# gildas-lormeau/zlib-streams-ts

Measured on AMD Instinct MI355X. Metric: uncompressed MB/s, deflate-raw L6, 4096x64KiB batch at 1/2/4/8 GPUs, higher is better.
Workload: dtype u8; 1 GPU; 4096 x 65536 B text-corpus streams split across the GPUs, deflate-raw level 6; global_streams=4096, streams_per_gpu=4096, stream_bytes=65536, level=6, format=deflate-raw, compressed_bytes=91855591, parallelism=dp1

## Files before the change

### zlib-streams-ts_amd/csrc/deflate_sweep.hip

```cpp
#include <hip/hip_runtime.h>
#include "zs_common.h"
#include "zs_kernels.h"
#include <type_traits>

#define ZS_SW_WIN_WORDS ((ZS_SEG_WPOS + 258u + 20u + 3u) / 4u + 2u)
#define ZS_SW_RING 128u
#ifndef ZS_SW_EXP
#define ZS_SW_EXP 0
#endif
#define ZS_SW_MW 320u

typedef __attribute__((address_space(3))) uint32_t zs_sw_lds_u32;
static __device__ __forceinline__ uint32_t sw_lds_addr(const void* p) {
  return (uint32_t)(uintptr_t)(const zs_sw_lds_u32*)p;
}

static __device__ __forceinline__ uint32_t sw_hash(uint32_t w) {
  return (((w & 0xffu) << 10) ^ (((w >> 8) & 0xffu) << 5) ^ ((w >> 16) & 0xffu)) & ZS_HASH_MASK;
}

#define ZS_BK_WPT (16384u / ZS_BK_THREADS)
#define ZS_BK_PPL (ZS_BK_THREADS / 64u)
#ifndef ZS_BK_PROF
#define ZS_BK_PROF 0
#endif
#if ZS_BK_PROF
__device__ unsigned long long zs_bk_stat[4];
extern "C" int zs_bucket_stats(unsigned long long* out) {
  return (int)hipMemcpyFromSymbol(out, HIP_SYMBOL(zs_bk_stat), sizeof(zs_bk_stat));
}
#define BK_MARK(i) do { if (threadIdx.x == 0) { const unsigned long long t_ = wall_clock64(); atomicAdd(&zs_bk_stat[i], t_ - bk_t); bk_t = t_; } } while (0)
#else
#define BK_MARK(i) do { } while (0)
#endif
#define ZS_BK_INFLIGHT 8
#define ZS_BK_CHUNK 2048u

template <bool ORD>
__global__ __launch_bounds__(ZS_BK_THREADS) void zs_k_bucket(const uint8_t* __restrict__ in,
                                                            const uint64_t* __restrict__ in_off,
                                                            const uint32_t* __restrict__ in_len,
                                                            const uint64_t* __restrict__ pos_base,
                                                            const zs_sweep_seg* __restrict__ segs,
                                                            uint16_t* __restrict__ members, uint2* __restrict__ mres) {
  __shared__ uint32_t cnt[16384];
  __shared__ uint32_t part[ZS_BK_THREADS];
  __shared__ uint32_t stg[ZS_BK_CHUNK / 4 + 2];
  __shared__ uint16_t q[2][ZS_BK_CHUNK];
  const zs_sweep_seg G = segs[blockIdx.x];
  const int s = (int)G.s;
  const uint32_t nrel = in_len[s] - G.base;
  const uint32_t tid = threadIdx.x;
  const uint8_t* src = in + in_off[s] + G.base;
  uint16_t* mem = members + G.mb;
  uint2* out = mres + pos_base[s] + G.base;
  const uint32_t m = nrel > 2 ? min(nrel - 2, G.ohi) : 0u;
  const uint32_t n = min(nrel, m + 2u);
  if (nrel - m <= 2u)
    for (uint32_t p = m + tid; p < nrel; p += ZS_BK_THREADS) out[p] = make_uint2(0, 0);
  if (m == 0) return;
  for (uint32_t i = tid; i < 16384 / 4; i += ZS_BK_THREADS) reinterpret_cast<uint4*>(cnt)[i] = make_uint4(0, 0, 0, 0);
  const bool aligned = ((uintptr_t)src & 3u) == 0;
#if ZS_BK_PROF
  unsigned long long bk_t = wall_clock64();
  if (threadIdx.x == 0) atomicAdd(&zs_bk_stat[3], 1ull);
#endif
  __syncthreads();
  {
    uint32_t w[5], nw[5];
    auto load5 = [&](uint32_t p0, uint32_t* x) __attribute__((always_inline)) {
#pragma unroll
      for (int k = 0; k < 5; k++) x[k] = zs_load_word(src, n, p0 + 16 * tid + 4 * k);
    };
    load5(0, nw);
    for (uint32_t p0 = 0; p0 < m; p0 += 16 * ZS_BK_THREADS) {
#pragma unroll
      for (int k = 0; k < 5; k++) w[k] = nw[k];
      if (p0 + 16 * ZS_BK_THREADS < m) load5(p0 + 16 * ZS_BK_THREADS, nw);
#pragma unroll
      for (uint32_t j = 0; j < 16; j++) {
        const uint32_t p = p0 + 16 * tid + j;
        const uint32_t h = sw_hash(__builtin_amdgcn_alignbyte(w[(j >> 2) + 1], w[j >> 2], j & 3u));
        if (p < m) atomicAdd(&cnt[h >> 1], 1u << (16u * (h & 1u)));
      }
    }
  }
  __syncthreads();
  BK_MARK(0);
  {
    uint32_t sum = 0;
    for (uint32_t j = 0; j < ZS_BK_WPT; j++) {
      const uint32_t w = cnt[ZS_BK_WPT * tid + ((j + tid) & (ZS_BK_WPT - 1u))];
      sum += (w & 0xffffu) + (w >> 16);
    }
    part[tid] = sum;
    __syncthreads();
    if (tid < 64) {
      uint32_t v[ZS_BK_PPL], t = 0;
#pragma unroll
      for (uint32_t j = 0; j < ZS_BK_PPL; j++) { v[j] = part[ZS_BK_PPL * tid + j]; t += v[j]; }
      uint32_t x = t;
#pragma unroll
      for (int d = 1; d < 64; d <<= 1) {
        const uint32_t y = __shfl_up(x, d, 64);
        if (tid >= (uint32_t)d) x += y;
      }
      uint32_t run = x - t;
#pragma unroll
      for (uint32_t j = 0; j < ZS_BK_PPL; j++) { part[ZS_BK_PPL * tid + j] = run; run += v[j]; }
    }
    __syncthreads();
    uint32_t run = part[tid];
    for (uint32_t j = 0; j < ZS_BK_WPT; j++) {
      const uint32_t w = cnt[ZS_BK_WPT * tid + j];
      const uint32_t lo = w & 0xffffu;
      cnt[ZS_BK_WPT * tid + j] = run | ((run + lo) << 16);
      run += lo + (w >> 16);
    }
  }
  __syncthreads();
  BK_MARK(1);
  const uint32_t wave = tid >> 6, lane = tid & 63u;
  constexpr uint32_t CW = ZS_BK_CHUNK / 4 / 64;
  uint32_t nxt[CW + 1];
  auto fetch = [&](uint32_t c0) {
#pragma unroll
    for (uint32_t i = 0; i <= CW; i++) {
      const uint32_t w = 64 * i + lane;
      const uint32_t at = c0 + 4 * w;
      uint32_t v = 0;
      if (w < ZS_BK_CHUNK / 4 + 2) {
        if (aligned && at + 4 <= n) v = *(const uint32_t*)(src + at);
        else
          for (uint32_t k = 0; k < 4; k++)
            if (at + k < n) v |= (uint32_t)src[at + k] << (8 * k);
      }
      nxt[i] = v;
    }
  };
  if (wave == 0) fetch(0);
  const uint32_t nch = (m + ZS_BK_CHUNK - 1) / ZS_BK_CHUNK;
  for (uint32_t c = 0; c <= nch; c++) {
    const uint32_t c0 = c * ZS_BK_CHUNK;
    if (wave == 0 && c < nch) {
      __builtin_amdgcn_s_waitcnt(0xc07f);
      __builtin_amdgcn_wave_barrier();
#pragma unroll
      for (uint32_t i = 0; i <= CW; i++)
        if (64 * i + lane < ZS_BK_CHUNK / 4 + 2) stg[64 * i + lane] = nxt[i];
      __builtin_amdgcn_s_waitcnt(0xc07f);
      __builtin_amdgcn_wave_barrier();
      if (c0 + ZS_BK_CHUNK < m) fetch(c0 + ZS_BK_CHUNK);
      const uint32_t c1 = min(m, c0 + ZS_BK_CHUNK);
      uint16_t* const qc = q[c & 1u];
      for (uint32_t g0 = c0; g0 < c1; g0 += 64 * ZS_BK_INFLIGHT) {
        uint32_t a[ZS_BK_INFLIGHT], v[ZS_BK_INFLIGHT], sh[ZS_BK_INFLIGHT], e[ZS_BK_INFLIGHT], hh[ZS_BK_INFLIGHT];
#pragma unroll
        for (int j = 0; j < ZS_BK_INFLIGHT; j++) {
          const uint32_t p = g0 + 64 * j + lane;
          const uint32_t o = p - c0;
          const uint32_t h = sw_hash(__builtin_amdgcn_alignbyte(stg[(o >> 2) + 1], stg[o >> 2], o & 3u));
          hh[j] = h;
          sh[j] = 16u * (h & 1u);
          a[j] = sw_lds_addr(&cnt[h >> 1]);
          v[j] = p < c1 ? 1u << sh[j] : 0u;
        }
        if (!ORD) {
#pragma unroll
          for (int j = 0; j < ZS_BK_INFLIGHT; j++) {
            const uint32_t p = g0 + 64 * j + lane;
            const uint32_t h = hh[j];
            const uint64_t mm = zs_wave_match(h, p < c1);
            const uint32_t rank = (uint32_t)__builtin_popcountll(mm & ((1ull << lane) - 1ull));
            const uint32_t lead = mm ? (uint32_t)__builtin_ctzll(mm) : lane;
            uint32_t old = 0;
            if (p < c1 && lead == lane)
              old = atomicAdd(&cnt[h >> 1], (uint32_t)__builtin_popcountll(mm) << sh[j]);
            old = (uint32_t)__builtin_amdgcn_ds_bpermute((int)(lead * 4u), (int)old);
            e[j] = old + (rank << sh[j]);
          }
        } else {
        asm volatile(
            "ds_add_rtn_u32 %0, %8, %16\n\t"
            "ds_add_rtn_u32 %1, %9, %17\n\t"
            "ds_add_rtn_u32 %2, %10, %18\n\t"
            "ds_add_rtn_u32 %3, %11, %19\n\t"
            "ds_add_rtn_u32 %4, %12, %20\n\t"
            "ds_add_rtn_u32 %5, %13, %21\n\t"
            "ds_add_rtn_u32 %6, %14, %22\n\t"
            "ds_add_rtn_u32 %7, %15, %23\n\t"
            "s_waitcnt lgkmcnt(0)"
            : "=&v"(e[0]), "=&v"(e[1]), "=&v"(e[2]), "=&v"(e[3]), "=&v"(e[4]), "=&v"(e[5]), "=&v"(e[6]), "=&v"(e[7])
            : "v"(a[0]), "v"(a[1]), "v"(a[2]), "v"(a[3]), "v"(a[4]), "v"(a[5]), "v"(a[6]), "v"(a[7]), "v"(v[0]),
              "v"(v[1]), "v"(v[2]), "v"(v[3]), "v"(v[4]), "v"(v[5]), "v"(v[6]), "v"(v[7])
            : "memory");
        }
#pragma unroll
        for (int j = 0; j < ZS_BK_INFLIGHT; j++) {
          const uint32_t p = g0 + 64 * j + lane;
          if (p < c1) qc[p - c0] = (uint16_t)(e[j] >> sh[j]);
        }
      }
    } else if (wave != 0 && c > 0) {
      const uint32_t b0 = c0 - ZS_BK_CHUNK, cnt1 = min(m, c0) - b0;
      const uint16_t* const qp = q[(c - 1) & 1u];
      for (uint32_t o = tid - 64u; o < cnt1; o += ZS_BK_THREADS - 64u) mem[qp[o]] = (uint16_t)(b0 + o);
    }
    __syncthreads();
  }
  BK_MARK(2);
}
template __global__ void zs_k_bucket<true>(const uint8_t*, const uint64_t*, const uint32_t*, const uint64_t*,
                                           const zs_sweep_seg*, uint16_t*, uint2*);
template __global__ void zs_k_bucket<false>(const uint8_t*, const uint64_t*, const uint32_t*, const uint64_t*,
                                            const zs_sweep_seg*, uint16_t*, uint2*);

static __device__ __forceinline__ uint32_t sw_word(const uint32_t* win, uint32_t off) {
  const uint32_t i = off >> 2;
  return __builtin_amdgcn_alignbyte(win[i + 1], win[i], off & 3u);
}

static __device__ __forceinline__ uint32_t sw_extend(const uint32_t* win, uint32_t p, uint32_t q, uint32_t maxc,
                                                     uint32_t from) {
  uint32_t k = from;
  while (k < maxc) {
    const uint32_t y = sw_word(win, q + k) ^ sw_word(win, p + k);
    if (y) { k += (uint32_t)(__builtin_ctz(y) >> 3); break; }
    k += 4;
  }
  return k < maxc ? k : maxc;
}

static __device__ __forceinline__ uint64_t sw_uniform(uint64_t x) {
  return ((uint64_t)(uint32_t)__builtin_amdgcn_readfirstlane((uint32_t)(x >> 32)) << 32) |
         (uint64_t)(uint32_t)__builtin_amdgcn_readfirstlane((uint32_t)x);
}

static __device__ __forceinline__ uint32_t max3(uint32_t a, uint32_t b, uint32_t c) {
  return max(max(a, b), c);
}

static __device__ __forceinline__ uint32_t sw_x7(uint32_t w) {
  const uint32_t b0 = w & 0xffu, b1 = (w >> 8) & 0xffu;
  return ((b0 >> 5) & 3u) | ((b1 & 7u) << 2) | (((b1 >> 5) & 3u) << 5);
}
template <bool A7>
struct SwSig;
template <>
struct SwSig<false> {
  static constexpr uint32_t LONG = 88u;
  static constexpr uint32_t THR0 = 23u;
  static constexpr uint32_t EXT = 11u;
  uint32_t a, b, c;
  __device__ __forceinline__ void own(const uint32_t* win, uint32_t p) {
    a = sw_word(win, p);
    b = sw_word(win, p + 4);
    c = (sw_word(win, p + 8) & 0x00ffffffu) | 0x01000000u;
  }
  static __device__ __forceinline__ uint4 rec(const uint32_t* win, uint32_t q, uint32_t w0) {
    return make_uint4(w0, sw_word(win, q + 4), sw_word(win, q + 8) & 0x00ffffffu, 0u);
  }
  __device__ __forceinline__ uint32_t mbits(uint32_t x, uint32_t y, uint32_t z) const {
    uint32_t f0, f1, f2;
    asm("v_ffbl_b32 %0, %1" : "=v"(f0) : "v"(x ^ a));
    asm("v_ffbl_b32 %0, %1\n\tv_add_u32_e64 %0, %0, 32 clamp" : "=&v"(f1) : "v"(y ^ b));
    asm("v_ffbl_b32 %0, %1\n\tv_add_u32_e32 %0, 64, %0" : "=&v"(f2) : "v"(z ^ c));
    return min(min(f0, f1), f2);
  }
  static __device__ __forceinline__ uint32_t len(uint32_t sigma) { return sigma; }
};
template <>
struct SwSig<true> {
  static constexpr uint32_t LONG = 64u;
  static constexpr uint32_t THR0 = 7u;
  static constexpr uint32_t EXT = 10u;
  uint32_t a, b;
  __device__ __forceinline__ void own(const uint32_t* win, uint32_t p) {
    a = sw_x7(sw_word(win, p)) | (sw_word(win, p + 3) << 8);
    b = sw_word(win, p + 6);
  }
  static __device__ __forceinline__ uint4 rec(const uint32_t* win, uint32_t q, uint32_t w0) {
    return make_uint4(sw_x7(w0) | (sw_word(win, q + 3) << 8), sw_word(win, q + 6), sw_word(win, q + EXT), 0u);
  }
  __device__ __forceinline__ uint32_t mbits(uint32_t x, uint32_t y, uint32_t) const {
    uint32_t f0, f1;
    asm("v_ffbl_b32 %0, %1" : "=v"(f0) : "v"(x ^ a));
    asm("v_ffbl_b32 %0, %1\n\tv_add_u32_e64 %0, %0, 32 clamp" : "=&v"(f1) : "v"(y ^ b));
    return min(min(f0, f1), 64u);
  }
  static __device__ __forceinline__ uint32_t len(uint32_t sigma) { return sigma ? sigma + 2u : 2u; }
};

struct SwRing {
  uint2 ab[2 * ZS_SW_RING];
  uint32_t c[2 * ZS_SW_RING];
  uint32_t key[2 * ZS_SW_RING];
};

#if ZS_SW_EXP & 64
__device__ unsigned long long zs_sw_stat[8];
#define SW_STAT(i, v) do { if ((threadIdx.x & 63u) == __builtin_ctzll(__builtin_amdgcn_read_exec())) atomicAdd(&zs_sw_stat[i], (unsigned long long)(v)); } while (0)
extern "C" int zs_sw_stats(unsigned long long* out) {
  return (int)hipMemcpyFromSymbol(out, HIP_SYMBOL(zs_sw_stat), sizeof(zs_sw_stat));
}
#else
#define SW_STAT(i, v) do { } while (0)
#endif

template <bool A7, bool MW>
static __device__ __forceinline__ void sw_body(const uint32_t* win, SwRing* R, uint16_t* mw, uint32_t* next,
                                               uint32_t n, uint32_t m, uint32_t olo, uint32_t ohi,
                                               const uint16_t* mem, uint2* out, int chain, int nice_cfg) {
  using Sig = SwSig<A7>;
  const uint32_t lane = threadIdx.x & 63u;
  const uint32_t budget = (uint32_t)chain, budget_s = (uint32_t)chain >> 2;
#if ZS_SW_EXP & 128
  const uint32_t sbud = 4u;
#else
  const uint32_t sbud = budget;
#endif
  const uint32_t nchunks = (m + 63) / 64;
  auto put_rec = [&](int j, uint4 r) {
    const uint32_t i = (uint32_t)j & (ZS_SW_RING - 1);
    R->ab[i] = make_uint2(r.x, r.y);
    R->ab[i + ZS_SW_RING] = make_uint2(r.x, r.y);
    R->c[i] = r.z;
    R->c[i + ZS_SW_RING] = r.z;
    R->key[i] = r.w;
    R->key[i + ZS_SW_RING] = r.w;
  };
  auto make_rec = [&](uint32_t q) -> uint4 {
    const uint32_t w0 = sw_word(win, q);
    uint4 r = Sig::rec(win, q, w0);
    r.w = (sw_hash(w0) << 16) | q;
    return r;
  };
  int mw0 = 0;
  auto load_rec_q = [&](int j, uint32_t q) {
    const bool in = j >= 0 && (uint32_t)j < m;
    if (MW && (uint32_t)(j - mw0) < ZS_SW_MW) mw[j - mw0] = (uint16_t)q;
    put_rec(j, in ? make_rec(q) : make_uint4(0, 0, 0, 0));
  };
  auto fetch = [&](int j) -> uint32_t { return j >= 0 && (uint32_t)j < m ? (uint32_t)mem[j] : 0u; };
  auto load_rec = [&](int j) { load_rec_q(j, fetch(j)); };
  auto member = [&](int j) -> uint32_t { return MW ? (uint32_t)mw[j - mw0] : (uint32_t)mem[j]; };
  auto rmbits = [&](const Sig& S, uint32_t slot) -> uint32_t {
    const uint2 ab = R->ab[slot];
    return S.mbits(ab.x, ab.y, A7 ? 0u : R->c[slot]);
  };
  auto claim = [&]() -> uint32_t {
    uint32_t c = 0;
    if (lane == 0) c = atomicAdd(next, 1u);
    return __builtin_amdgcn_readfirstlane(c);
  };
  uint32_t c = claim();
  uint32_t pf_p = fetch((int)(64 * c + lane)), pf_b = fetch((int)(64 * c + lane) - 64);
  for (;;) {
    if (c >= nchunks) break;
    const uint32_t cn = claim();
    const int k0 = (int)(64 * c);
    const int k = k0 + (int)lane;
    const bool mem_ok = (uint32_t)k < m;
    SW_STAT(0, 1);
    const uint32_t p = pf_p, qb = pf_b;
    if (cn < nchunks) {
      pf_p = fetch((int)(64 * cn + lane));
      pf_b = fetch((int)(64 * cn + lane) - 64);
    }
    c = cn;
    const bool own = mem_ok && p >= olo && p < ohi;
    if (__builtin_amdgcn_ballot_w64(own) == 0) continue;
    mw0 = k0 - (int)sbud;
    if (MW) mw[k - mw0] = (uint16_t)p;
    Sig S;
    S.own(win, p);
    const uint32_t h = sw_hash(sw_word(win, p));
    const uint32_t look = n - p;
    const uint32_t maxc = look < ZS_MAX_MATCH ? look : ZS_MAX_MATCH;
    const uint32_t nice = look < (uint32_t)nice_cfg ? look : (uint32_t)nice_cfg;
    const bool tail = maxc <= 12u;
    const uint32_t long_m = tail ? 0xffffu : Sig::LONG;
    const uint32_t limit = p > ZS_MAX_DIST ? p - ZS_MAX_DIST : 0u;
    const uint32_t khead = (h << 16) | (limit > 1u ? limit : 1u);
    const uint32_t klim = (h << 16) | limit;
    __builtin_amdgcn_s_waitcnt(0xc07f);
    __builtin_amdgcn_wave_barrier();
    put_rec(k, mem_ok ? make_rec(p) : make_uint4(0, 0, 0, 0));
#if ZS_SW_EXP & 256
    put_rec(k - 64, make_uint4(qb, qb, qb, 0));
#else
    load_rec_q(k - 64, qb);
#endif
    __builtin_amdgcn_s_waitcnt(0xc07f);
    __builtin_amdgcn_wave_barrier();

    uint32_t thr = Sig::THR0, thr_s = Sig::THR0;
    uint32_t bt = 0, bt_s = 0;
    uint32_t lthr = 7u, lbt = 0, lthr_s = 7u, lbt_s = 0;
    const uint32_t own_ext = sw_word(win, p + Sig::EXT);
    uint64_t alive_m = 0;
    uint32_t head = 0;
    auto score = [&](uint32_t mb, uint32_t u) -> uint32_t { return (mb & ~7u) | (7u - u); };
    auto fold = [&](uint32_t gm, uint32_t t0, const uint32_t* sc, uint32_t cnt, uint32_t base)
        __attribute__((always_inline)) {
#if ZS_SW_EXP & 4096
      const bool up = gm > thr;
      thr = max(thr, gm | 7u);
      bt = up ? t0 + 7u - (gm & 7u) : bt;
#else
      const bool up = gm > (thr | 7u);
      thr = up ? gm : thr;
      bt = up ? t0 : bt;
#endif
#if ZS_SW_EXP & 32
      if (0) {
#else
      if (__builtin_expect(__builtin_amdgcn_ballot_w64(gm >= long_m) != 0, 0)) {
#endif
        SW_STAT(3, 1);
        if (gm >= long_m && (lthr >> 3) < nice) {
          uint32_t gl = 0;
#if ZS_SW_EXP & 1024
#pragma unroll
          for (uint32_t u = 0; u < 8; u++) {
            if (u < cnt && sc[u] >= long_m) {
#else
          uint32_t lm = 0;
#pragma unroll
          for (uint32_t u = 0; u < 8; u++) lm |= (u < cnt && sc[u] >= long_m) ? 1u << u : 0u;
          while (lm) {
            const uint32_t u = (uint32_t)__builtin_ctz(lm);
            lm &= lm - 1u;
            {
#endif
              const uint32_t x = (A7 ? R->c[base - t0 - u]
                                     : sw_word(win, (R->key[base - t0 - u] & 0xffffu) + Sig::EXT)) ^ own_ext;
              uint32_t len = x ? Sig::EXT + ((uint32_t)__builtin_ctz(x) >> 3)
                               : sw_extend(win, p, R->key[base - t0 - u] & 0xffffu, maxc, Sig::EXT + 4u);
              len = min(min(len, maxc), nice);
              gl = max(gl, (len << 3) | (7u - u));
            }
          }
          const bool lup = gl > lthr;
          lthr = max(lthr, gl | 7u);
          lbt = lup ? t0 + 7u - (gl & 7u) : lbt;
        }
      }
    };
    bool snapped = budget_s <= 1u;
    auto snap = [&](uint32_t t1) __attribute__((always_inline)) {
      if (t1 == budget_s) {
        thr_s = thr;
        bt_s = bt;
        lthr_s = lthr;
        lbt_s = lbt;
        snapped = true;
      }
    };
    const uint32_t base0 = (((uint32_t)(k - 64)) & (ZS_SW_RING - 1)) + 64u;
    {
      const uint32_t key = R->key[base0 - 1u];
      bool a1 = false;
      uint32_t sc[1] = {0};
      if (own && key >= khead) {
        a1 = true;
        head = 1u | ((p - (key & 0xffffu)) == ZS_MAX_DIST ? 0x8000u : 0u);
        sc[0] = score(rmbits(S, base0 - 1u), 0);
      }
      alive_m = __builtin_amdgcn_ballot_w64(a1);
      fold(sc[0], 1u, sc, 1u, base0);
      snap(1u);
    }
    auto mstep = [&](uint32_t slot, uint32_t u, uint64_t& lm) -> uint32_t {
      const uint32_t key = R->key[slot];
      asm("v_cmp_gt_u32_e64 %0, %1, %2" : "=s"(lm) : "v"(key), "v"(klim));
      lm &= alive_m;
      const uint32_t v = score(rmbits(S, slot), u);
      uint32_t r;
      asm("v_cndmask_b32_e64 %0, 0, %1, %2" : "=v"(r) : "v"(v), "s"(lm));
      return r;
    };
    if (sbud >= 4u) {
      uint32_t sc[3];
      uint64_t lm = 0;
#pragma unroll
      for (uint32_t u = 0; u < 3; u++) sc[u] = mstep(base0 - 2u - u, u, lm);
      alive_m = sw_uniform(lm);
      fold(max3(sc[0], sc[1], sc[2]), 2u, sc, 3u, base0);
      snap(4u);
    }
    auto group_fast = [&](uint32_t base, uint32_t t0, auto G, bool live) __attribute__((always_inline)) {
      constexpr uint32_t N = decltype(G)::value;
      const uint32_t lo = base - t0 - (N - 1u);
      const uint2* const A = R->ab + lo;
      const uint32_t* const C = R->c + lo;
      uint32_t sc[N];
#pragma unroll
      for (uint32_t u = 0; u < N; u++) {
        const uint2 ab = A[N - 1u - u];
        sc[u] = score(S.mbits(ab.x, ab.y, A7 ? 0u : C[N - 1u - u]), u);
      }
      uint32_t gm;
      if constexpr (N == 8)
        gm = max(max3(sc[0], sc[1], sc[2]), max3(sc[3], sc[4], max3(sc[5], sc[6], sc[7])));
      else
        gm = max3(sc[0], sc[1], max(sc[2], sc[3]));
      fold(live ? gm : 0u, t0, sc, N, base);
    };
    auto group_masked = [&](uint32_t base, uint32_t t0, auto G) __attribute__((always_inline)) {
      constexpr uint32_t N = decltype(G)::value;
#if ZS_SW_EXP & 8192
      uint32_t sc[8];
      uint64_t lm = 0, last = 0;
#pragma unroll
      for (uint32_t u = 0; u < 8; u++) {
        sc[u] = 0u;
        if (u < N) {
          sc[u] = mstep(base - t0 - u, u, lm);
          last = lm;
        }
      }
      alive_m = sw_uniform(last);
      fold(max(max3(sc[0], sc[1], sc[2]), max3(sc[3], sc[4], max3(sc[5], sc[6], sc[7]))), t0, sc, N, base);
#else
      const uint32_t lo = base - t0 - (N - 1u);
      const uint2* const A = R->ab + lo;
      const uint32_t* const C = R->c + lo;
      const uint32_t* const K = R->key + lo;
      uint32_t sc[N], key[N];
      uint2 ab[N];
#pragma unroll
      for (uint32_t u = 0; u < N; u++) {
        key[u] = K[N - 1u - u];
        ab[u] = A[N - 1u - u];
      }
      uint64_t lm = 0;
#pragma unroll
      for (uint32_t u = 0; u < N; u++) {
        asm("v_cmp_gt_u32_e64 %0, %1, %2" : "=s"(lm) : "v"(key[u]), "v"(klim));
        lm &= alive_m;
        const uint32_t v = score(S.mbits(ab[u].x, ab[u].y, A7 ? 0u : C[N - 1u - u]), u);
        asm("v_cndmask_b32_e64 %0, 0, %1, %2" : "=v"(sc[u]) : "v"(v), "s"(lm));
      }
      alive_m = sw_uniform(lm);
      uint32_t gm;
      if constexpr (N == 8)
        gm = max(max3(sc[0], sc[1], sc[2]), max3(sc[3], sc[4], max3(sc[5], sc[6], sc[7])));
      else
        gm = max3(sc[0], sc[1], max(sc[2], sc[3]));
      fold(gm, t0, sc, N, base);
#endif
    };
    using G8 = std::integral_constant<uint32_t, 8>;
    using G4 = std::integral_constant<uint32_t, 4>;
    auto run = [&](uint32_t base, uint32_t ta, uint32_t tb) __attribute__((always_inline)) {
#if !(ZS_SW_EXP & 16384)
      auto last_of = [&](uint32_t t0) __attribute__((always_inline)) {
        uint32_t t1 = t0 + 7u <= tb ? t0 + 7u : t0 + 3u;
        if (t0 <= budget_s && t1 > budget_s) t1 = budget_s;
        return t1;
      };
      if (ta > tb) return;
      uint32_t t0 = ta, t1 = last_of(ta);
      uint32_t kl = R->key[base - t1];
      while (alive_m) {
        const bool mine = ((alive_m >> lane) & 1u) != 0;
        const uint64_t last_live = __builtin_amdgcn_ballot_w64(mine && kl > klim);
        const uint32_t n0 = t1 + 1u, n1 = n0 <= tb ? last_of(n0) : t1;
        kl = R->key[base - n1];
        if (last_live == alive_m) {
          SW_STAT(1, 1);
          SW_STAT(4, t1 - t0 + 1u);
          if (t1 - t0 == 7u) group_fast(base, t0, G8{}, mine);
          else group_fast(base, t0, G4{}, mine);
        } else {
          SW_STAT(2, 1);
          SW_STAT(4, t1 - t0 + 1u);
          if (t1 - t0 == 7u) group_masked(base, t0, G8{});
          else group_masked(base, t0, G4{});
        }
        snap(t1);
        if (n0 > tb) break;
        t0 = n0;
        t1 = n1;
      }
#else
      for (uint32_t t0 = ta; t0 <= tb && alive_m;) {
        uint32_t t1 = t0 + 7u <= tb ? t0 + 7u : t0 + 3u;
        if (t0 <= budget_s && t1 > budget_s) t1 = budget_s;
        const bool mine = ((alive_m >> lane) & 1u) != 0;
        const uint64_t last_live = __builtin_amdgcn_ballot_w64(mine && R->key[base - t1] > klim);
#if ZS_SW_EXP & 4
        if (0) {
#elif ZS_SW_EXP & 16
        if (1) {
#else
        if (last_live == alive_m) {
#endif
          SW_STAT(1, 1);
          SW_STAT(4, t1 - t0 + 1u);
          if (t1 - t0 == 7u) group_fast(base, t0, G8{}, mine);
          else group_fast(base, t0, G4{}, mine);
        } else {
          SW_STAT(2, 1);
          SW_STAT(4, t1 - t0 + 1u);
          if (t1 - t0 == 7u) group_masked(base, t0, G8{});
          else group_masked(base, t0, G4{});
        }
        snap(t1);
        t0 = t1 + 1u;
      }
#endif
    };
    for (uint32_t b = 0; sbud > 4u && alive_m; b++) {
      if (b >= 1) {
        __builtin_amdgcn_s_waitcnt(0xc07f);
        __builtin_amdgcn_wave_barrier();
        load_rec(k - 64 * (int)(b + 1));
        __builtin_amdgcn_s_waitcnt(0xc07f);
        __builtin_amdgcn_wave_barrier();
      }
      const uint32_t ta = b == 0 ? 5u : 64u * b + 1u;
      const uint32_t tb = min(64u * b + 64u, sbud);
      const uint32_t base = (((uint32_t)(k - 64 * (int)b - 64)) & (ZS_SW_RING - 1)) + 64u * b + 64u;
      run(base, ta, tb);
      if (tb >= sbud) break;
    }
    if (!snapped) {
      thr_s = thr;
      bt_s = bt;
      lthr_s = lthr;
      lbt_s = lbt;
    }
    __builtin_amdgcn_s_waitcnt(0xc07f);
    __builtin_amdgcn_wave_barrier();
    if (own) {
      uint32_t rx = 0, ry = 0;
      if (head) {
        uint32_t L = 2, D = 0, Ls = 2, Ds = 0;
        if (tail) {
          uint32_t b = 2u << 16, bs = 2u << 16;
          for (uint32_t t = 1; t <= budget && (int)t <= k; t++) {
            const uint32_t q = t <= sbud ? member(k - (int)t) : (uint32_t)mem[k - (int)t];
            const uint32_t key = (sw_hash(sw_word(win, q)) << 16) | q;
            if (t == 1u ? key < khead : key <= klim) break;
            uint32_t len = 12;
            for (uint32_t o = 0; o < 12u; o += 4) {
              const uint32_t y = sw_word(win, q + o) ^ sw_word(win, p + o);
              if (y) { len = o + (uint32_t)(__builtin_ctz(y) >> 3); break; }
            }
            const uint32_t sc = ((len < maxc ? len : maxc) << 16) | (0xffffu - t);
            b = max(b, sc);
            if (t <= budget_s) bs = max(bs, sc);
          }
          L = b >> 16;
          D = L > 2u ? p - (uint32_t)mem[k - (int)(0xffffu - (b & 0xffffu))] : 0u;
          Ls = bs >> 16;
          Ds = Ls > 2u ? p - (uint32_t)mem[k - (int)(0xffffu - (bs & 0xffffu))] : 0u;
        } else {
#if ZS_SW_EXP & 4096
          const uint32_t tb = bt, tb_s = bt_s;
#else
          const uint32_t tb = bt + 7u - (thr & 7u), tb_s = bt_s + 7u - (thr_s & 7u);
#endif
          if (bt) {
            L = Sig::len(thr >> 3);
            D = p - member(k - (int)tb);
          }
          if (bt_s) {
            Ls = Sig::len(thr_s >> 3);
            Ds = tb_s == tb ? D : p - member(k - (int)tb_s);
          }
          auto long_of = [&](uint32_t lt, uint32_t t, uint32_t& len, uint32_t& dist) {
            const uint32_t q = member(k - (int)t);
            len = lt >> 3;
            if (len >= nice) len = sw_extend(win, p, q, maxc, Sig::EXT);
            dist = p - q;
          };
          if (lbt) long_of(lthr, lbt, L, D);
          if (lbt_s) {
            if (lbt_s == lbt) {
              Ls = L;
              Ds = D;
            } else {
              long_of(lthr_s, lbt_s, Ls, Ds);
            }
          }
        }
        rx = (L << 16) | (L > 2u ? D : 0u) | (head & 0x8000u);
        ry = (Ls << 16) | (Ls > 2u ? Ds : 0u);
      }
#if ZS_SW_EXP & 512
      if (rx == 0x12345678u) out[p] = make_uint2(rx, ry);
#else
      out[p] = make_uint2(rx, ry);
#endif
    }
  }
}

__global__ __launch_bounds__(1024) void zs_k_sweep(const uint8_t* __restrict__ in, const uint64_t* __restrict__ in_off,
                                                   const uint32_t* __restrict__ in_len,
                                                   const uint64_t* __restrict__ pos_base,
                                                   const zs_sweep_seg* __restrict__ segs,
                                                   const uint16_t* __restrict__ members, uint2* __restrict__ mres,
                                                   int chain, int nice_cfg) {
  __shared__ __attribute__((aligned(16))) SwRing ring[16];
  __shared__ __attribute__((aligned(16))) uint32_t win[ZS_SW_WIN_WORDS];
  __shared__ uint16_t mwin[16][ZS_SW_MW];
  __shared__ uint32_t next;
  const zs_sweep_seg G = segs[blockIdx.x];
  const int s = (int)G.s;
  const uint32_t n = in_len[s] - G.base;
  if (n < 3) return;
  const uint32_t m = min(n - 2, G.ohi);
  const uint8_t* src = in + in_off[s] + G.base;
  uint32_t hi = 0;
  if ((((uintptr_t)src) & 15u) == 0) {
    for (uint32_t i = threadIdx.x; 4 * i < ZS_SW_WIN_WORDS; i += 1024) {
      const uint32_t b = 16 * i;
      uint4 v;
      if (b + 16 <= n) v = ((const uint4*)src)[i];
      else {
        uint32_t t[4] = {0, 0, 0, 0};
        for (uint32_t k = 0; k < 16; k++)
          if (b + k < n) t[k >> 2] |= (uint32_t)src[b + k] << (8 * (k & 3));
        v = make_uint4(t[0], t[1], t[2], t[3]);
      }
      hi |= v.x | v.y | v.z | v.w;
      if (4 * i + 3 < ZS_SW_WIN_WORDS) *(uint4*)(win + 4 * i) = v;
      else for (uint32_t k = 0; 4 * i + k < ZS_SW_WIN_WORDS; k++) win[4 * i + k] = (&v.x)[k];
    }
  } else {
    for (uint32_t i = threadIdx.x; i < ZS_SW_WIN_WORDS; i += 1024) {
      uint32_t v = 0;
      for (uint32_t k = 0; k < 4; k++)
        if (4 * i + k < n) v |= (uint32_t)src[4 * i + k] << (8 * k);
      hi |= v;
      win[i] = v;
    }
  }
  if (threadIdx.x == 0) next = 0;
  const bool a7 = !__syncthreads_or((hi & 0x80808080u) != 0);
  SwRing* const R = &ring[threadIdx.x >> 6];
  const uint16_t* mem = members + G.mb;
  uint2* out = mres + pos_base[s] + G.base;
  uint16_t* const mw = mwin[threadIdx.x >> 6];
  const uint32_t olo = G.olo, ohi = G.ohi;
  if (chain + 64 <= (int)ZS_SW_MW) {
    if (a7) sw_body<true, true>(win, R, mw, &next, n, m, olo, ohi, mem, out, chain, nice_cfg);
    else sw_body<false, true>(win, R, mw, &next, n, m, olo, ohi, mem, out, chain, nice_cfg);
  } else {
    if (a7) sw_body<true, false>(win, R, mw, &next, n, m, olo, ohi, mem, out, chain, nice_cfg);
    else sw_body<false, false>(win, R, mw, &next, n, m, olo, ohi, mem, out, chain, nice_cfg);
  }
}
```

Before: 19460 MB/s.

## Claim chunk runs per wave and reuse persistent 3-block candidate ring

Each wave now claims a run of consecutive 64-position chunks with one atomic, instead of one chunk per atomic. It keeps a persistent 3-block LDS ring of candidate records across consecutive chunks, so the previous blocks' records are reused rather than rebuilt. Member positions are read back from the ring keys instead of a separate member window. The own-position record is computed once and reused for the signature, hash and extension word. This aims to cut redundant record construction, LDS writes, global member fetches and atomic traffic, at the cost of more complex slot indexing, coarser work balancing, and a path that is limited to chain lengths up to 128.

```diff
diff --git a/zlib-streams-ts_amd/csrc/deflate_sweep.hip b/zlib-streams-ts_amd/csrc/deflate_sweep.hip
--- a/zlib-streams-ts_amd/csrc/deflate_sweep.hip
+++ b/zlib-streams-ts_amd/csrc/deflate_sweep.hip
@@ -1,6 +1,7 @@
 #include <hip/hip_runtime.h>
 #include "zs_common.h"
 #include "zs_kernels.h"
+#include "zs_sweep_ring.h"
 #include <type_traits>
 
 #define ZS_SW_WIN_WORDS ((ZS_SEG_WPOS + 258u + 20u + 3u) / 4u + 2u)
@@ -9,6 +10,7 @@
 #define ZS_SW_EXP 0
 #endif
 #define ZS_SW_MW 320u
+#define ZS_SW_RUN_CAP ((((ZS_SW_EXP) >> 16) & 31u) ? (((ZS_SW_EXP) >> 16) & 31u) : 16u)
 
 typedef __attribute__((address_space(3))) uint32_t zs_sw_lds_u32;
 static __device__ __forceinline__ uint32_t sw_lds_addr(const void* p) {
@@ -296,6 +298,11 @@
   uint32_t c[2 * ZS_SW_RING];
   uint32_t key[2 * ZS_SW_RING];
 };
+struct SwRingP {
+  uint2 ab[ZS_SWR_SLOTS + ZS_SWR_MIRROR];
+  uint32_t c[ZS_SWR_SLOTS + ZS_SWR_MIRROR];
+  uint32_t key[ZS_SWR_SLOTS + ZS_SWR_MIRROR];
+};
 
 #if ZS_SW_EXP & 64
 __device__ unsigned long long zs_sw_stat[8];
@@ -307,11 +314,13 @@
 #define SW_STAT(i, v) do { } while (0)
 #endif
 
-template <bool A7, bool MW>
-static __device__ __forceinline__ void sw_body(const uint32_t* win, SwRing* R, uint16_t* mw, uint32_t* next,
+template <bool A7, bool MW, bool PR>
+static __device__ __forceinline__ void sw_body(const uint32_t* win, void* ringp, uint16_t* mw, uint32_t* next,
                                                uint32_t n, uint32_t m, uint32_t olo, uint32_t ohi,
                                                const uint16_t* mem, uint2* out, int chain, int nice_cfg) {
   using Sig = SwSig<A7>;
+  using Ring = std::conditional_t<PR, SwRingP, SwRing>;
+  Ring* const R = (Ring*)ringp;
   const uint32_t lane = threadIdx.x & 63u;
   const uint32_t budget = (uint32_t)chain, budget_s = (uint32_t)chain >> 2;
 #if ZS_SW_EXP & 128
@@ -329,6 +338,18 @@
     R->key[i] = r.w;
     R->key[i + ZS_SW_RING] = r.w;
   };
+  auto put_blk = [&](int blk, uint4 r) {
+    const uint32_t i = zs_swr_block_slot(blk) + lane;
+    R->ab[i] = make_uint2(r.x, r.y);
+    R->c[i] = r.z;
+    R->key[i] = r.w;
+    if (zs_swr_mirrored(blk)) {
+      R->ab[i + ZS_SWR_SLOTS] = make_uint2(r.x, r.y);
+      R->c[i + ZS_SWR_SLOTS] = r.z;
+      R->key[i + ZS_SWR_SLOTS] = r.w;
+    }
+  };
+  auto at = [&](uint32_t base, uint32_t t) -> uint32_t { return base - t; };
   auto make_rec = [&](uint32_t q) -> uint4 {
     const uint32_t w0 = sw_word(win, q);
     uint4 r = Sig::rec(win, q, w0);
@@ -343,7 +364,15 @@
   };
   auto fetch = [&](int j) -> uint32_t { return j >= 0 && (uint32_t)j < m ? (uint32_t)mem[j] : 0u; };
   auto load_rec = [&](int j) { load_rec_q(j, fetch(j)); };
-  auto member = [&](int j) -> uint32_t { return MW ? (uint32_t)mw[j - mw0] : (uint32_t)mem[j]; };
+  int cc = 0;
+  auto build_blk = [&](int blk, uint32_t q) {
+    const int j = 64 * blk + (int)lane;
+    put_blk(blk, j >= 0 && (uint32_t)j < m ? make_rec(q) : make_uint4(0, 0, 0, 0));
+  };
+  auto member = [&](int j) -> uint32_t {
+    if constexpr (PR) return R->key[zs_swr_member_slot(cc, lane, 64u * (uint32_t)cc + lane - (uint32_t)j)] & 0xffffu;
+    return MW ? (uint32_t)mw[j - mw0] : (uint32_t)mem[j];
+  };
   auto rmbits = [&](const Sig& S, uint32_t slot) -> uint32_t {
     const uint2 ab = R->ab[slot];
     return S.mbits(ab.x, ab.y, A7 ? 0u : R->c[slot]);
@@ -353,11 +382,35 @@
     if (lane == 0) c = atomicAdd(next, 1u);
     return __builtin_amdgcn_readfirstlane(c);
   };
-  uint32_t c = claim();
+  auto claim_run = [&](uint32_t& c0, uint32_t& c1) {
+    uint32_t a = 0, r = 0;
+    if (lane == 0) {
+      const uint32_t cur = __hip_atomic_load(next, __ATOMIC_RELAXED, __HIP_MEMORY_SCOPE_WORKGROUP);
+      r = zs_swr_run_len(cur < nchunks ? nchunks - cur : 0u, ZS_SW_RUN_CAP);
+      a = atomicAdd(next, r);
+    }
+    c0 = __builtin_amdgcn_readfirstlane(a);
+    c1 = min(c0 + (uint32_t)__builtin_amdgcn_readfirstlane(r), nchunks);
+  };
+  uint32_t c, ce = 0;
+  if constexpr (PR) claim_run(c, ce);
+  else c = claim();
   uint32_t pf_p = fetch((int)(64 * c + lane)), pf_b = fetch((int)(64 * c + lane) - 64);
+  zs_swr_range vr = zs_swr_empty();
+  bool fresh_n = true;
   for (;;) {
     if (c >= nchunks) break;
-    const uint32_t cn = claim();
+    const bool fresh = fresh_n;
+    uint32_t cn, cen = ce;
+    if constexpr (PR) {
+      cn = c + 1u;
+      fresh_n = cn >= ce;
+      if (fresh_n) claim_run(cn, cen);
+      if (fresh) vr = zs_swr_empty();
+    } else {
+      cn = claim();
+    }
+    cc = (int)c;
     const int k0 = (int)(64 * c);
     const int k = k0 + (int)lane;
     const bool mem_ok = (uint32_t)k < m;
@@ -365,16 +418,27 @@
     const uint32_t p = pf_p, qb = pf_b;
     if (cn < nchunks) {
       pf_p = fetch((int)(64 * cn + lane));
-      pf_b = fetch((int)(64 * cn + lane) - 64);
+      if (!PR || fresh_n) pf_b = fetch((int)(64 * cn + lane) - 64);
     }
     c = cn;
+    ce = cen;
     const bool own = mem_ok && p >= olo && p < ohi;
-    if (__builtin_amdgcn_ballot_w64(own) == 0) continue;
+    if (__builtin_amdgcn_ballot_w64(own) == 0) {
+      vr = zs_swr_empty();
+      continue;
+    }
     mw0 = k0 - (int)sbud;
     if (MW) mw[k - mw0] = (uint16_t)p;
+    const uint4 rown = PR && mem_ok ? make_rec(p) : make_uint4(0, 0, 0, 0);
     Sig S;
-    S.own(win, p);
-    const uint32_t h = sw_hash(sw_word(win, p));
+    if constexpr (PR) {
+      S.a = rown.x;
+      S.b = rown.y;
+      if constexpr (!A7) S.c = rown.z | 0x01000000u;
+    } else {
+      S.own(win, p);
+    }
+    const uint32_t h = PR ? rown.w >> 16 : sw_hash(sw_word(win, p));
     const uint32_t look = n - p;
     const uint32_t maxc = look < ZS_MAX_MATCH ? look : ZS_MAX_MATCH;
     const uint32_t nice = look < (uint32_t)nice_cfg ? look : (uint32_t)nice_cfg;
@@ -385,19 +449,28 @@
     const uint32_t klim = (h << 16) | limit;
     __builtin_amdgcn_s_waitcnt(0xc07f);
     __builtin_amdgcn_wave_barrier();
-    put_rec(k, mem_ok ? make_rec(p) : make_uint4(0, 0, 0, 0));
+    if constexpr (PR) {
+      put_blk(cc, rown);
+      vr = zs_swr_push(vr, cc);
+      if (!zs_swr_has(vr, cc - 1)) {
+        build_blk(cc - 1, fresh ? qb : fetch(k - 64));
+        vr = zs_swr_extend(vr, cc - 1);
+      }
+    } else {
+      put_rec(k, mem_ok ? make_rec(p) : make_uint4(0, 0, 0, 0));
 #if ZS_SW_EXP & 256
-    put_rec(k - 64, make_uint4(qb, qb, qb, 0));
-#else
-    load_rec_q(k - 64, qb);
-#endif
+      put_rec(k - 64, make_uint4(qb, qb, qb, 0));
+#else
+      load_rec_q(k - 64, qb);
+#endif
+    }
     __builtin_amdgcn_s_waitcnt(0xc07f);
     __builtin_amdgcn_wave_barrier();
 
     uint32_t thr = Sig::THR0, thr_s = Sig::THR0;
     uint32_t bt = 0, bt_s = 0;
     uint32_t lthr = 7u, lbt = 0, lthr_s = 7u, lbt_s = 0;
-    const uint32_t own_ext = sw_word(win, p + Sig::EXT);
+    const uint32_t own_ext = PR && A7 ? rown.z : sw_word(win, p + Sig::EXT);
     uint64_t alive_m = 0;
     uint32_t head = 0;
     auto score = [&](uint32_t mb, uint32_t u) -> uint32_t { return (mb & ~7u) | (7u - u); };
@@ -433,10 +506,10 @@
             lm &= lm - 1u;
             {
 #endif
-              const uint32_t x = (A7 ? R->c[base - t0 - u]
-                                     : sw_word(win, (R->key[base - t0 - u] & 0xffffu) + Sig::EXT)) ^ own_ext;
+              const uint32_t ls = at(base, t0 + u);
+              const uint32_t x = (A7 ? R->c[ls] : sw_word(win, (R->key[ls] & 0xffffu) + Sig::EXT)) ^ own_ext;
               uint32_t len = x ? Sig::EXT + ((uint32_t)__builtin_ctz(x) >> 3)
-                               : sw_extend(win, p, R->key[base - t0 - u] & 0xffffu, maxc, Sig::EXT + 4u);
+                               : sw_extend(win, p, R->key[ls] & 0xffffu, maxc, Sig::EXT + 4u);
               len = min(min(len, maxc), nice);
               gl = max(gl, (len << 3) | (7u - u));
             }
@@ -457,15 +530,15 @@
         snapped = true;
       }
     };
-    const uint32_t base0 = (((uint32_t)(k - 64)) & (ZS_SW_RING - 1)) + 64u;
+    const uint32_t base0 = PR ? zs_swr_base(cc, 0u) + lane : (((uint32_t)(k - 64)) & (ZS_SW_RING - 1)) + 64u;
     {
-      const uint32_t key = R->key[base0 - 1u];
+      const uint32_t key = R->key[at(base0, 1u)];
       bool a1 = false;
       uint32_t sc[1] = {0};
       if (own && key >= khead) {
         a1 = true;
         head = 1u | ((p - (key & 0xffffu)) == ZS_MAX_DIST ? 0x8000u : 0u);
-        sc[0] = score(rmbits(S, base0 - 1u), 0);
+        sc[0] = score(rmbits(S, at(base0, 1u)), 0);
       }
       alive_m = __builtin_amdgcn_ballot_w64(a1);
       fold(sc[0], 1u, sc, 1u, base0);
@@ -484,14 +557,14 @@
       uint32_t sc[3];
       uint64_t lm = 0;
 #pragma unroll
-      for (uint32_t u = 0; u < 3; u++) sc[u] = mstep(base0 - 2u - u, u, lm);
+      for (uint32_t u = 0; u < 3; u++) sc[u] = mstep(at(base0, 2u + u), u, lm);
       alive_m = sw_uniform(lm);
       fold(max3(sc[0], sc[1], sc[2]), 2u, sc, 3u, base0);
       snap(4u);
     }
     auto group_fast = [&](uint32_t base, uint32_t t0, auto G, bool live) __attribute__((always_inline)) {
       constexpr uint32_t N = decltype(G)::value;
-      const uint32_t lo = base - t0 - (N - 1u);
+      const uint32_t lo = at(base, t0 + (N - 1u));
       const uint2* const A = R->ab + lo;
       const uint32_t* const C = R->c + lo;
       uint32_t sc[N];
@@ -516,14 +589,14 @@
       for (uint32_t u = 0; u < 8; u++) {
         sc[u] = 0u;
         if (u < N) {
-          sc[u] = mstep(base - t0 - u, u, lm);
+          sc[u] = mstep(at(base, t0 + u), u, lm);
           last = lm;
         }
       }
       alive_m = sw_uniform(last);
       fold(max(max3(sc[0], sc[1], sc[2]), max3(sc[3], sc[4], max3(sc[5], sc[6], sc[7]))), t0, sc, N, base);
 #else
-      const uint32_t lo = base - t0 - (N - 1u);
+      const uint32_t lo = at(base, t0 + (N - 1u));
       const uint2* const A = R->ab + lo;
       const uint32_t* const C = R->c + lo;
       const uint32_t* const K = R->key + lo;
@@ -562,12 +635,12 @@
       };
       if (ta > tb) return;
       uint32_t t0 = ta, t1 = last_of(ta);
-      uint32_t kl = R->key[base - t1];
+      uint32_t kl = R->key[at(base, t1)];
       while (alive_m) {
         const bool mine = ((alive_m >> lane) & 1u) != 0;
         const uint64_t last_live = __builtin_amdgcn_ballot_w64(mine && kl > klim);
         const uint32_t n0 = t1 + 1u, n1 = n0 <= tb ? last_of(n0) : t1;
-        kl = R->key[base - n1];
+        kl = R->key[at(base, n1)];
         if (last_live == alive_m) {
           SW_STAT(1, 1);
           SW_STAT(4, t1 - t0 + 1u);
@@ -589,7 +662,7 @@
         uint32_t t1 = t0 + 7u <= tb ? t0 + 7u : t0 + 3u;
         if (t0 <= budget_s && t1 > budget_s) t1 = budget_s;
         const bool mine = ((alive_m >> lane) & 1u) != 0;
-        const uint64_t last_live = __builtin_amdgcn_ballot_w64(mine && R->key[base - t1] > klim);
+        const uint64_t last_live = __builtin_amdgcn_ballot_w64(mine && R->key[at(base, t1)] > klim);
 #if ZS_SW_EXP & 4
         if (0) {
 #elif ZS_SW_EXP & 16
@@ -613,16 +686,22 @@
 #endif
     };
     for (uint32_t b = 0; sbud > 4u && alive_m; b++) {
-      if (b >= 1) {
+      if (b >= 1 && (!PR || !zs_swr_has(vr, cc - (int)b - 1))) {
         __builtin_amdgcn_s_waitcnt(0xc07f);
         __builtin_amdgcn_wave_barrier();
-        load_rec(k - 64 * (int)(b + 1));
+        if constexpr (PR) {
+          build_blk(cc - (int)b - 1, fetch(k - 64 * (int)(b + 1)));
+          vr = zs_swr_extend(vr, cc - (int)b - 1);
+        } else {
+          load_rec(k - 64 * (int)(b + 1));
+        }
         __builtin_amdgcn_s_waitcnt(0xc07f);
         __builtin_amdgcn_wave_barrier();
       }
       const uint32_t ta = b == 0 ? 5u : 64u * b + 1u;
       const uint32_t tb = min(64u * b + 64u, sbud);
-      const uint32_t base = (((uint32_t)(k - 64 * (int)b - 64)) & (ZS_SW_RING - 1)) + 64u * b + 64u;
+      const uint32_t base = PR ? zs_swr_base(cc, b) + lane
+                               : (((uint32_t)(k - 64 * (int)b - 64)) & (ZS_SW_RING - 1)) + 64u * b + 64u;
       run(base, ta, tb);
       if (tb >= sbud) break;
     }
@@ -705,9 +784,10 @@
                                                    const zs_sweep_seg* __restrict__ segs,
                                                    const uint16_t* __restrict__ members, uint2* __restrict__ mres,
                                                    int chain, int nice_cfg) {
-  __shared__ __attribute__((aligned(16))) SwRing ring[16];
+  constexpr uint32_t RING_BYTES = 16u * sizeof(SwRing), MWIN_BYTES = 16u * ZS_SW_MW * sizeof(uint16_t);
+  static_assert(16u * sizeof(SwRingP) <= RING_BYTES + MWIN_BYTES, "the persistent rings must fit the old ones' LDS");
+  __shared__ __attribute__((aligned(16))) uint8_t rmem[RING_BYTES + MWIN_BYTES];
   __shared__ __attribute__((aligned(16))) uint32_t win[ZS_SW_WIN_WORDS];
-  __shared__ uint16_t mwin[16][ZS_SW_MW];
   __shared__ uint32_t next;
   const zs_sweep_seg G = segs[blockIdx.x];
   const int s = (int)G.s;
@@ -742,16 +822,23 @@
   }
   if (threadIdx.x == 0) next = 0;
   const bool a7 = !__syncthreads_or((hi & 0x80808080u) != 0);
-  SwRing* const R = &ring[threadIdx.x >> 6];
+  const uint32_t wave = threadIdx.x >> 6;
   const uint16_t* mem = members + G.mb;
   uint2* out = mres + pos_base[s] + G.base;
-  uint16_t* const mw = mwin[threadIdx.x >> 6];
   const uint32_t olo = G.olo, ohi = G.ohi;
+  if (chain <= (int)ZS_SWR_MAX_CHAIN) {
+    SwRingP* const R = reinterpret_cast<SwRingP*>(rmem) + wave;
+    if (a7) sw_body<true, false, true>(win, R, nullptr, &next, n, m, olo, ohi, mem, out, chain, nice_cfg);
+    else sw_body<false, false, true>(win, R, nullptr, &next, n, m, olo, ohi, mem, out, chain, nice_cfg);
+    return;
+  }
+  SwRing* const R = reinterpret_cast<SwRing*>(rmem) + wave;
+  uint16_t* const mw = reinterpret_cast<uint16_t*>(rmem + RING_BYTES) + wave * ZS_SW_MW;
   if (chain + 64 <= (int)ZS_SW_MW) {
-    if (a7) sw_body<true, true>(win, R, mw, &next, n, m, olo, ohi, mem, out, chain, nice_cfg);
-    else sw_body<false, true>(win, R, mw, &next, n, m, olo, ohi, mem, out, chain, nice_cfg);
+    if (a7) sw_body<true, true, false>(win, R, mw, &next, n, m, olo, ohi, mem, out, chain, nice_cfg);
+    else sw_body<false, true, false>(win, R, mw, &next, n, m, olo, ohi, mem, out, chain, nice_cfg);
   } else {
-    if (a7) sw_body<true, false>(win, R, mw, &next, n, m, olo, ohi, mem, out, chain, nice_cfg);
-    else sw_body<false, false>(win, R, mw, &next, n, m, olo, ohi, mem, out, chain, nice_cfg);
-  }
-}
+    if (a7) sw_body<true, false, false>(win, R, mw, &next, n, m, olo, ohi, mem, out, chain, nice_cfg);
+    else sw_body<false, false, false>(win, R, mw, &next, n, m, olo, ohi, mem, out, chain, nice_cfg);
+  }
+}
diff --git a/zlib-streams-ts_amd/csrc/zs_sweep_ring.h b/zlib-streams-ts_amd/csrc/zs_sweep_ring.h
--- /dev/null
+++ b/zlib-streams-ts_amd/csrc/zs_sweep_ring.h
@@ -0,0 +1,59 @@
+#ifndef ZS_SWEEP_RING_H
+#define ZS_SWEEP_RING_H
+#include <stdint.h>
+
+#if defined(__HIPCC__)
+#define ZS_SWR_FN static __host__ __device__ __forceinline__
+#else
+#define ZS_SWR_FN static inline
+#endif
+
+#define ZS_SWR_BLOCKS 3u
+#define ZS_SWR_SLOTS 192u
+#define ZS_SWR_MIRROR 64u
+#define ZS_SWR_MAX_CHAIN 128u
+#define ZS_SWR_RUN_DIV 32u
+
+ZS_SWR_FN uint32_t zs_swr_block_slot(int32_t b) { return 64u * ((uint32_t)(b + 3) % ZS_SWR_BLOCKS); }
+
+ZS_SWR_FN int zs_swr_mirrored(int32_t b) { return zs_swr_block_slot(b) == 0u; }
+
+ZS_SWR_FN uint32_t zs_swr_base(int32_t c, uint32_t s) {
+  return zs_swr_block_slot(c - (int32_t)s - 1) + 64u * s + 64u;
+}
+
+ZS_SWR_FN uint32_t zs_swr_member_slot(int32_t c, uint32_t l, uint32_t t) {
+  const uint32_t s = zs_swr_block_slot(c - 2) + 128u + l - t;
+  return s >= ZS_SWR_SLOTS ? s - ZS_SWR_SLOTS : s;
+}
+
+typedef struct { int32_t lo, hi; } zs_swr_range;
+
+ZS_SWR_FN zs_swr_range zs_swr_empty(void) {
+  zs_swr_range r;
+  r.lo = 1;
+  r.hi = 0;
+  return r;
+}
+ZS_SWR_FN int zs_swr_has(zs_swr_range r, int32_t b) { return r.lo <= b && b <= r.hi; }
+
+ZS_SWR_FN zs_swr_range zs_swr_push(zs_swr_range r, int32_t c) {
+  if (r.lo > r.hi || r.hi != c - 1) {
+    r.lo = c;
+  } else if (r.lo < c - 2) {
+    r.lo = c - 2;
+  }
+  r.hi = c;
+  return r;
+}
+ZS_SWR_FN zs_swr_range zs_swr_extend(zs_swr_range r, int32_t b) {
+  r.lo = b;
+  return r;
+}
+
+ZS_SWR_FN uint32_t zs_swr_run_len(uint32_t left, uint32_t cap) {
+  const uint32_t r = left / ZS_SWR_RUN_DIV;
+  return r < 1u ? 1u : (r > cap ? cap : r);
+}
+
+#endif
```

New measurement: 19880 MB/s, median of 6. +2.1%, better.
